# etzinis/sudo_rm_rf

Hardware: AMD Instinct MI355X
Metric: separated-seconds/sec (4s@8kHz mixtures), Improved-U16/512, 1->8 MI355X (higher is better)
Workload: dtype f32 (1x1 convs: fp32 operands split into bf16 hi+lo, 3 bf16 MFMAs per product, fp32 accumulate)

## Files before the change

### include/sudormrf_hip.h

```cpp
#ifndef SUDORMRF_HIP_H
#define SUDORMRF_HIP_H

#include <stddef.h>

#ifdef __cplusplus
extern "C" {
#endif

#define SRF_ABI_VERSION 19

#define SRF_STAT_BUCKETS 64

#define SRF_OK 0
#define SRF_EINVAL (-1)
#define SRF_EHIP (-2)
#define SRF_EWORKSPACE (-3)

#define SRF_VARIANT_IMPROVED 0
#define SRF_VARIANT_GROUPCOMM 1
#define SRF_VARIANT_CAUSAL 2

typedef struct srf_config {
  int variant;
  int in_audio_channels;
// ... 42 lines not shown
  SRF_DBG_GEMM_128_ONE_TILE_PER_BLOCK = 2048,
  SRF_DBG_WGRAD_NO_XCD_MAP = 4096,
  SRF_DBG_GEMM_256_SWAP_FORMS = 8192,
  SRF_DBG_TRAIN_BF16X3 = 16384,
  SRF_DBG_NO_FUSED_TAIL = 32768,
  SRF_DBG_BWD_NO_FUSED_HEAD = 1 << 16,
  SRF_DBG_PYR_PASS1_ROWS_PER_WAVE = 1 << 17,
  SRF_DBG_WGRAD_NO_WIDE_TILE = 1 << 18,
  SRF_DBG_WGRAD_128_MASKED = 1 << 19,
  SRF_DBG_WGRAD_SHORT_CHUNKS = 1 << 20,
  SRF_DBG_PAIR_PERSISTENT = 1 << 21,
  SRF_DBG_TAC_VALU = 1 << 22,
  SRF_DBG_PAIR_FULL_DRAIN = 1 << 23,
  SRF_DBG_TAC_GENERIC = 1 << 24,
  SRF_DBG_WGRAD_ONE_CHAIN_FOLD = 1 << 25,
  SRF_DBG_TAC_LANES_4TILES = 1 << 26,
  SRF_DBG_GEMM_128_POINTER_LOADS = 1 << 27,
  SRF_DBG_TRAIN_FWD_SPLIT_BF16 = 1 << 28,
  SRF_DBG_BWD_DW_CHUNKED = 1 << 29,
  SRF_DBG_BWD_GLN_SCALAR = 1 << 30,
  SRF_DBG_TRAIN_FWD_EXACT_MFMA = -2147483647 - 1
};
void srf_set_debug_flags(int flags);
#endif

int srf_plan_create(const srf_config* cfg, int batch, int T, srf_plan** out);
void srf_plan_destroy(srf_plan* plan);
size_t srf_plan_workspace_bytes(const srf_plan* plan);
int srf_plan_num_params(const srf_plan* plan);
int srf_plan_frames(const srf_plan* plan);
int srf_plan_padded_length(const srf_plan* plan);
int srf_plan_num_launches(const srf_plan* plan);

int srf_forward(const srf_plan* plan, const float* const* params, int num_params,
                const float* wav, float* out, void* workspace, size_t workspace_bytes, void* stream);

int srf_plan_ragged_supported(const srf_plan* plan);
size_t srf_plan_ragged_workspace_bytes(const srf_plan* plan);
int srf_forward_ragged(const srf_plan* plan, const float* const* params, int num_params, const float* wav,
                       const int* lengths , float* out, void* workspace, size_t workspace_bytes,
                       void* stream);

int srf_separate(const srf_plan* plan, const float* const* params, int num_params, const float* wav, float* out,
                 float* stats, int mixture_consistency, void* workspace, size_t workspace_bytes, void* stream);

int srf_separate_ragged(const srf_plan* plan, const float* const* params, int num_params, const float* wav,
// ... 316 lines not shown
```

### sudo_rm_rf_amd/_lib.py

```python
import ctypes as C
import os
import threading

import torch

_PKG = os.path.dirname(os.path.abspath(__file__))
LIB_PATH = os.environ.get("SRF_LIB") or os.path.join(_PKG, "libsudormrf_hip.so")
ABI_VERSION = 19
RAGGED_MAX_BATCH = 128
STAT_BUCKETS = 64

SRF_OK = 0
VARIANT_IMPROVED, VARIANT_GROUPCOMM, VARIANT_CAUSAL, VARIANT_ATTENTIVE, VARIANT_ATTENTIVE_V3, VARIANT_ORIGINAL = 0, 1, 2, 3, 4, 5
ATT_MAX_LEN = 5000
SOFTMAX_MASK_MAX_SOURCES = 16


class SrfError(RuntimeError):
    pass


class srf_config(C.Structure):
    _fields_ = [(n, C.c_int) for n in (
        "variant", "in_audio_channels", "out_channels", "in_channels", "num_blocks",
        "upsampling_depth", "enc_kernel_size", "enc_num_basis", "num_sources", "group_size")]


class srf_norm(C.Structure):
    _fields_ = [("sums", C.c_void_p), ("gamma", C.c_void_p), ("beta", C.c_void_p), ("prelu", C.c_void_p)]


class srf_stream_row(C.Structure):
    _fields_ = [("slot", C.c_int), ("n", C.c_int)]


_vp, _i, _sz, _l = C.c_void_p, C.c_int, C.c_size_t, C.c_long
_PROTOS = {
    "srf_abi_version": (_i, []),
    "srf_last_error": (C.c_char_p, []),
    "srf_set_kernel_mode": (None, [_i]),
    "srf_get_kernel_mode": (_i, []),
    "srf_profile_begin": (_i, [_vp]),
    "srf_profile_end": (_i, [_vp, C.POINTER(_i)]),
    "srf_profile_get": (_i, [_i, C.POINTER(C.c_char_p), C.POINTER(C.c_float)]),
    "srf_profile_timeline": (_i, [_i, C.POINTER(C.c_char_p), C.POINTER(C.c_float), C.POINTER(_i)]),
    "srf_plan_create": (_i, [C.POINTER(srf_config), _i, _i, C.POINTER(_vp)]),
    "srf_plan_destroy": (None, [_vp]),
    "srf_plan_workspace_bytes": (_sz, [_vp]),
    "srf_plan_num_params": (_i, [_vp]),
    "srf_plan_frames": (_i, [_vp]),
    "srf_plan_padded_length": (_i, [_vp]),
    "srf_plan_num_launches": (_i, [_vp]),
    "srf_forward": (_i, [_vp, C.POINTER(_vp), _i, _vp, _vp, _vp, _sz, _vp]),
    "srf_debug_fetch": (_i, [_vp, _vp, _i, _vp, _sz, _vp]),
    "srf_encoder": (_i, [_vp, _vp, _vp, _vp, _i, _i, _i, _i, _i, _i, _vp]),
    "srf_gln_stats": (_i, [_vp, _vp, _i, _l, _vp]),
    "srf_gln_apply": (_i, [_vp, _vp, C.POINTER(srf_norm), _i, _i, _i, _vp]),
    "srf_gln_apply_add": (_i, [_vp, _vp, _vp, C.POINTER(srf_norm), _i, _i, _i, _vp]),
    "srf_pw_conv": (_i, [_vp, _vp, _vp, _vp, _i, _i, _i, _i, C.POINTER(srf_norm), _vp, _vp, _i, _vp, _i, _vp]),
    "srf_set_debug_flags": (None, [_i]),
    "srf_packed_pw_weight_bytes": (_sz, [_i, _i]),
    "srf_pack_pw_weights": (_i, [C.POINTER(_vp), C.POINTER(_vp), C.POINTER(_i), C.POINTER(_i), _i, _vp]),
    "srf_pw_conv_packed": (_i, [_vp, _vp, _vp, _vp, _vp, _i, _i, _i, _i, C.POINTER(srf_norm), _vp, _vp, _i, _vp, _i, _vp]),
    "srf_pw_conv_pair_supported": (_i, [_i, _i, _i, _i, _i]),
    "srf_pw_conv_pair": (_i, [_vp, _vp, _vp, _vp, C.POINTER(srf_norm), _vp, _vp, _vp, _vp, _vp, _i, _i, _i, _i, _i, _vp]),
    "srf_pw_conv_pair_packed3_supported": (_i, [_i, _i, _i, _i, _i]),
    "srf_pw_conv_pair_packed3": (_i, [_vp, _vp, _vp, _vp, C.POINTER(srf_norm), _vp, _vp, _vp, _vp, _vp, _i, _i, _i, _i, _i, _vp]),
    "srf_packed3_pw_weight_bytes": (_sz, [_i, _i]),
    "srf_pack3_pw_weights": (_i, [C.POINTER(_vp), C.POINTER(_vp), C.POINTER(_i), C.POINTER(_i), _i, _vp]),
    "srf_pack3_forget": (None, [_vp]),
    "srf_pw_conv_packed3": (_i, [_vp, _vp, _vp, _vp, _vp, _i, _i, _i, _i, C.POINTER(srf_norm), _vp, _vp, _vp]),
    "srf_pit_sisdr_work_bytes": (_sz, [_i, _i]),
    "srf_perm_inv_sisdr_work_bytes": (_sz, [_i, _i]),
    "srf_perm_inv_sisdr": (_i, [_vp, _vp, _vp, _i, _i, _i, _i, C.c_double, _vp, _vp, _vp, _vp, _vp]),
    "srf_pit_sisdr_forward": (_i, [_vp, _vp, _i, _i, _i, C.c_float, _vp, _vp, _vp, _vp]),
    "srf_pit_sdr_forward": (_i, [_vp, _vp, _i, _i, _i, C.c_float, _i, _i, _i, _vp, _vp, _vp, _vp]),
    "srf_pit_sisdr_match": (_i, [_vp, _i, _i, _vp, _vp]),
    "srf_pit_sisdr_backward": (_i, [_vp, _vp, _i, _i, _i, C.c_float, _vp, _vp, _vp, _vp, _vp]),
    "srf_zeroref_snr_work_bytes": (_sz, [_i, _i, _i]),
    "srf_zeroref_snr_forward": (_i, [_vp, _vp, _i, _i, _i, _i, C.c_float, C.c_float, C.c_float, _vp, _vp, _vp, _vp, _vp]),
    "srf_zeroref_snr_backward": (_i, [_vp, _vp, _i, _i, _i, _vp, _vp, _i, _vp, _vp]),
    "srf_stab_sisdr_work_bytes": (_sz, [_i, _i]),
    "srf_stab_sisdr": (_i, [_vp, _vp, _i, _i, _i, _i, _i, _i, _i, C.c_double, _vp, _vp, _vp, _vp]),
# ... 197 lines not shown
```

### sudo_rm_rf_amd/csrc/srf_api.hip

```cpp
#include <string.h>

#include <atomic>
#include <mutex>
#include <new>
#include <vector>

#include "srf_plan.h"

static thread_local char g_err[512] = "";
static std::atomic<int> g_kernel_mode{0};

void srf_set_error(const char* fmt, ...) {
  va_list ap;
  va_start(ap, fmt);
  vsnprintf(g_err, sizeof(g_err), fmt, ap);
  va_end(ap);
}
static thread_local int g_kernel_mode_override = -1;
int srf_kernel_mode() { return g_kernel_mode_override >= 0 ? g_kernel_mode_override : g_kernel_mode.load(std::memory_order_relaxed); }
int srf_kernel_mode_override(int mode) {
  const int prev = g_kernel_mode_override;
  g_kernel_mode_override = mode;
  return prev;
}
static std::atomic<int> g_debug_flags{0};
int srf_debug_flags() { return g_debug_flags.load(std::memory_order_relaxed); }
extern "C" void srf_set_debug_flags(int f) { g_debug_flags.store(f, std::memory_order_relaxed); }

static std::mutex g_dev_mu;
static int g_dev_cus[SRF_MAX_DEVICES];
static long g_dev_occ[SRF_MAX_DEVICES][SRF_OCC_SLOTS];
static bool g_dev_occ_set[SRF_MAX_DEVICES][SRF_OCC_SLOTS];

int srf_current_device() {
  int dev = 0;
  return hipGetDevice(&dev) == hipSuccess ? dev : -1;
}
int srf_device_cus() {
  const int dev = srf_current_device();
  if (dev < 0 || dev >= SRF_MAX_DEVICES) return 256;
  std::lock_guard<std::mutex> lk(g_dev_mu);
  if (!g_dev_cus[dev]) {
    hipDeviceProp_t prop;
    g_dev_cus[dev] = hipGetDeviceProperties(&prop, dev) == hipSuccess ? prop.multiProcessorCount : 256;
  }
  return g_dev_cus[dev];
}
long srf_device_cached(int slot, long (*compute)(void*), void* arg) {
  const int dev = srf_current_device();
  if (dev < 0 || dev >= SRF_MAX_DEVICES || slot < 0 || slot >= SRF_OCC_SLOTS) return compute(arg);
// ... 398 lines not shown
}
static int step_pair(const Ragged* rg, const float* x, const void* w1_packed, const float* bias1, float* y, const srf_norm* in_norm,
                     const float* residual, const void* w2_packed, const float* bias2, float* y2, double* out_sums2, int Bt, int Cin1,
                     int Cmid, int Cout2, int L, void* stream) {
  return rg ? srf_pw_conv_pair_ragged(x, w1_packed, bias1, y, in_norm, residual, w2_packed, bias2, y2, out_sums2, Bt, Cin1, Cmid, Cout2,
                                      L, rg->frames, stream)
            : srf_pw_conv_pair(x, w1_packed, bias1, y, in_norm, residual, w2_packed, bias2, y2, out_sums2, Bt, Cin1, Cmid, Cout2, L,
                               stream);
}
static int step_tac(const Ragged* rg, const float* x, float* q, const float* const* params, int Bt, int G, int n, int H, int L,
                    double* out_sums, void* stream) {
  return rg ? srf_tac_ragged(x, q, params, Bt, G, n, H, L, out_sums, rg->frames, stream)
            : srf_tac(x, q, params, Bt, G, n, H, L, out_sums, stream);
}
static int step_preadd(const Ragged* rg, int G, const float* x, const float* q, const srf_norm* qnorm, float* u, const float* w,
                       const float* bias, float* y, int Bg, int Cin, int Cout, int L, double* out_sums, void* stream) {
  return rg ? srf_pw_conv_small_ragged(x, w, bias, y, Bg, Cin, Cout, L, nullptr, nullptr, out_sums, q, qnorm, u, rg->frames, G, stream)
            : srf_pw_conv_preadd(x, q, qnorm, u, w, bias, y, Bg, Cin, Cout, L, out_sums, (hipStream_t)stream);
}
static int step_pyramid(const Ragged* rg, int G, const float* y1, float* merged, const srf_norm* in_norm, const SrfBlock<const float>& b,
                        int Bg, int C, int L, int D, void* scratch, double* out_sums, void* stream) {
  return rg ? srf_pyramid_ragged_rows(y1, merged, in_norm, b.lv_w, b.lv_b, b.lv_g, b.lv_be, Bg, C, L, D, scratch, out_sums, rg->frames, G,
                                      stream)
            : srf_pyramid(y1, merged, in_norm, b.lv_w, b.lv_b, b.lv_g, b.lv_be, Bg, C, L, D, scratch, out_sums, stream);
}
static int step_overlap_add(const Ragged* rg, const float* z, float* out, int Bt, int Co, int K, int L, int T, int nparts,
                            const float* wav_stats, const float* wav, int mc, hipStream_t st) {
  return rg ? srf_overlap_add_launch(z, out, Bt, Co, K, L, T, nparts, wav_stats, wav, mc, st, &rg->lens_t, &rg->frames_t)
            : srf_overlap_add_launch(z, out, Bt, Co, K, L, T, nparts, wav_stats, wav, mc, st);
}

static int forward_walk(const srf_plan* p, const float* const* P, const float* wav, float* out, void* workspace,
                        const float* wav_stats, int mixture_consistency, const Ragged* rg, void* stream) {
  const srf_config& c = p->cfg;
  const bool gc = c.variant == SRF_VARIANT_GROUPCOMM;
  const int G = gc ? c.group_size : 1;
  const int D = c.upsampling_depth, U = c.num_blocks, N = c.enc_num_basis, K = c.enc_kernel_size;
  const int Bt = p->Bt, L = p->L, Bg = p->Bg, nB = p->nB, nC = p->nC;
  char* ws = (char*)workspace;
  hipStream_t st = (hipStream_t)stream;
  auto fptr = [&](size_t o) { return (float*)(ws + o); };
  double* stats = (double*)(ws + p->off_stats);
  int rc;

  rc = srf_zero_launch(stats, p->stats_bytes, st);
  if (rc) return rc;
  const bool use_pack = rg || plan_use_pack(p);
// ... 384 lines not shown
```

### sudo_rm_rf_amd/csrc/srf_common.h

```cpp
#pragma once
#include <hip/hip_runtime.h>
#include <stdarg.h>
#include <stdio.h>
#include <atomic>
#include <initializer_list>
#define SRF_DIAGNOSTICS 1
#include "../../include/sudormrf_hip.h"

#define SRF_WAVE 64
#define SRF_MAX_DEPTH 8

void srf_set_error(const char* fmt, ...);
int srf_kernel_mode();
int srf_kernel_mode_override(int mode);
int srf_debug_flags();
static inline bool srf_dbg(int mask) { return (srf_debug_flags() & mask) != 0; }
bool srf_profiling();
void srf_prof_hold(int delta);
void srf_prof_mark(const char* name, hipStream_t st);
#define SRF_MAX_DEVICES 64
int srf_current_device();
int srf_device_cus();
#define SRF_OCC_SLOTS 16
enum SrfOccSlot { SRF_OCC_PYR_PASS1_CH16 = 0, SRF_OCC_PYR_PASS1_CH32 = 1 };
long srf_device_cached(int slot, long (*compute)(void*), void* arg);

template <auto Kernel, typename... Args>
static inline bool srf_launch_lds(int max_lds, dim3 grid, dim3 block, size_t lds, hipStream_t st, const Args&... args) {
  static std::atomic<bool> raised[SRF_MAX_DEVICES];
  const int dev = srf_current_device();
  const bool known = dev >= 0 && dev < SRF_MAX_DEVICES;
  if (!known || !raised[dev].load(std::memory_order_acquire)) {
    if (hipFuncSetAttribute((const void*)Kernel, hipFuncAttributeMaxDynamicSharedMemorySize, max_lds) != hipSuccess) return false;
    if (known) raised[dev].store(true, std::memory_order_release);
  }
  hipLaunchKernelGGL(Kernel, grid, block, lds, st, args...);
  return true;
}

// ... 205 lines not shown
```

### sudo_rm_rf_amd/csrc/srf_internal.h

```cpp
#pragma once
#include "srf_common.h"

#define SRF_CAUSAL_TAPS 11
#define SRF_CAUSAL_KW 21

struct SrfFrames {
  int n[SRF_RAGGED_MAX_BATCH];
};
__device__ __forceinline__ int srf_frames_of(int) { return 0; }
__device__ __forceinline__ int srf_frames2_of(int) { return 0; }
template <typename... R>
__device__ __forceinline__ int srf_frames_of(int g, const SrfFrames& f, const R&...) { return f.n[g]; }
__device__ __forceinline__ int srf_frames2_of(int g, const SrfFrames&, const SrfFrames& f2) { return f2.n[g]; }
__device__ __forceinline__ int srf_frames_of(int row, const SrfFrames& f, int rows_per_example) { return f.n[row / rows_per_example]; }
int srf_frames_table(const char* what, const int* frames, int groups, int L, SrfFrames* out);

int srf_transpose_launch(const float* w, float* wt, int Ci, int M, hipStream_t st);
int srf_overlap_add_launch(const float* z, float* out, int Bt, int Co, int K, int L, int T, int nparts, const float* stats,
                           const float* wav, int mc, hipStream_t st, const SrfFrames* lens = nullptr,
                           const SrfFrames* frames = nullptr);
int srf_wav_stats_ragged_launch(const float* wav, const SrfFrames& lens, float* stats, int rows, int T, hipStream_t st);

int srf_zero_launch(void* p, size_t bytes, hipStream_t st);
int srf_decoder_impl(const float* v, const float* w, float* out, int Bt, int Ci, int Co, int K, int L, int T, float* scratch,
// ... 19 lines not shown

int srf_causal_scale_many(const float* const* src, float* const* dst, const long* n, const float* const* dscale,
                          const float* hscale, int count, hipStream_t st);

int srf_causal_merge_act(const float* const* d, const float* const* prelu, int D, float* y, int Bt, int C, int L, hipStream_t st);
int srf_causal_gain_fold(float* const* dw, float* const* db, const float* const* w, const float* const* b,
                         const float* const* gain, float* const* dgain, const float* alpha, int nw, int nb, int count,
                         hipStream_t st);
int srf_causal_enc_scatter(const float* src, float* dst, int N, int A, int K, hipStream_t st);
size_t srf_causal_prelu_bwd_scratch_floats();
int srf_causal_prelu_bwd(const float* gout, const float* x, const float* slope, float* gx, float* dslope, long n, float* scratch,
                         hipStream_t st);

template <typename T>
struct SrfBlock;
struct SrfSlots;
int srf_pyramid_per_level(const float* y1, float* const* lv, float* merged, const SrfBlock<const float>& b, const SrfSlots& s,
                          int Bg, int nC, int L, int D, void* stream);

bool srf_pyramid_reg_supported(int L, int D);
int srf_pyramid_impl(const float* y1, float* merged, const srf_norm* in_norm, const float* const* w,
                     const float* const* bias, const float* const* gamma, const float* const* beta, int groups, int C,
                     int L, int D, void* scratch, double* out_sums, float* const* lv_out, double* const* lv_sums,
                     void* stream);

void srf_pw_prefer_paired(bool on);
bool srf_pw_conv_preadd_supported(int Cin, int Cout, int L, const void* const* ptrs, int nptrs);
int srf_pw_conv_preadd(const float* x, const float* q, const srf_norm* qnorm, float* u, const float* w, const float* bias,
                       float* y, int Bt, int Cin, int Cout, int L, double* out_sums, hipStream_t st);
bool srf_mask_decode_supported(int Bt, int Cin, int Cout, int L, int M);
size_t srf_mask_decode_pack_bytes(int Cout);
int srf_mask_decode_pack(const float* wd, void* dst, int Ci, int M, hipStream_t st);
int srf_mask_decode(const float* x, const float* w, const void* w_packed, const float* bias, const float* prelu,
                    const float* mul, int mul_channels, const void* wd_packed, float* zpart, int Bt, int Cin, int Cout, int L,
                    int M, hipStream_t st);
int srf_pack_pw_weights_transposed(const float* const* w, void* const* packed, const int* Cout, const int* Cin, int n,
                                   hipStream_t st);
bool srf_pw_packed_only(const void* w_packed, const float* x, int Bt, int Cin, int Cout, int L);
bool srf_train_three_parts_override(bool on);
int srf_pw_data_grad(const float* g, const float* w, const void* wT_packed, float* wt, const float* zero_bias, float* gx, int Bt,
                     int Cin, int Cout, int L, const float* skip, hipStream_t st);

bool srf_x3w_supported(int Bt, int pro);
bool srf_x3w_shape_supported(int Cin, int Cout, int L);
size_t srf_x3w_packed_bytes(int Cout, int Cin);
int srf_x3w_pack_launch(const float* const* w, char* const* dst, const int* Cout, const int* Cin, int n, hipStream_t st);
int srf_x3w_pack2_launch(const float* const* w, char* const* dst, char* const* dst16, const int* Cout, const int* Cin, int n,
// ... 44 lines not shown
```

### sudo_rm_rf_amd/csrc/srf_pyr.h

```cpp
#pragma once
#include "srf_internal.h"

struct PyrRegArgs {
  const float* y1;
  float* d0;
  float* merged;
  SrfNormDev in_norm;
  const float* in_mr;
  double in_inv_count;
  const float* w[SRF_MAX_DEPTH];
  const float* bias[SRF_MAX_DEPTH];
  const float* gamma[SRF_MAX_DEPTH];
  const float* beta[SRF_MAX_DEPTH];
  const float* lvl;
  double* mom;
  double* out_sums;
  int rows;
  int rpw;
  int C, L, D, tiles, own;
  float* lv_out[SRF_MAX_DEPTH];
  int save = 0;
};

int srf_pyramid_reg_launch(PyrRegArgs a, bool moments, long rows, hipStream_t st, const SrfFrames* frames = nullptr,
                           int rows_per_example = 1);
```

### sudo_rm_rf_amd/csrc/srf_pyramid.hip

```cpp
#include "srf_pyr.h"

struct PyrArgs {
  const float* y1;
  float* merged;
  SrfNormDev in_norm;
  double in_inv_count;
  const float* w[SRF_MAX_DEPTH];
  const float* bias[SRF_MAX_DEPTH];
  const float* gamma[SRF_MAX_DEPTH];
  const float* beta[SRF_MAX_DEPTH];
  const float* lvl;
  const float* in_mr;
  float* d0;
  double* mom;
  double* out_sums;
  long rows;
  int C, L, D;
};

__device__ __forceinline__ float srf_dot5(const float* w, float x0, float x1, float x2, float x3, float x4,
                                          float init) {
  return fmaf(w[4], x4, fmaf(w[3], x3, fmaf(w[2], x2, fmaf(w[1], x1, fmaf(w[0], x0, init)))));
}

// ... 693 lines not shown
  t->TS = best;
  t->tiles = L / best;
  int h = 0;
  for (int k = SRF_MAX_DEPTH - 1; k >= 0; --k) {
    if (k >= D) {
      t->h[k] = 0;
      continue;
    }
    t->h[k] = (k == D - 1) ? 0 : 2 * h + 4;
    h = t->h[k];
  }
  const int len0 = best + 2 * t->h[0] + 8;
  int lv = 0;
  for (int k = 1; k < D; ++k) lv += (best >> k) + 2 * t->h[k] + 8;
  const int lenA = lv > len0 ? lv : len0;
  t->wave_floats = len0 + ((lenA + 3) & ~3) + 8 * SRF_MAX_DEPTH;
  return (size_t)t->wave_floats * 4 * sizeof(float) <= 64 * 1024;
}


int srf_pyramid_impl(const float* y1, float* merged, const srf_norm* in_norm, const float* const* w,
                     const float* const* bias, const float* const* gamma, const float* const* beta, int groups, int C,
                     int L, int D, void* scratch, double* out_sums, float* const* lv_out, double* const* lv_sums,
                     void* stream);

extern "C" int srf_pyramid(const float* y1, float* merged, const srf_norm* in_norm,
                           const float* const* w, const float* const* bias, const float* const* gamma,
                           const float* const* beta, int groups, int C, int L, int D, void* scratch,
                           double* out_sums, void* stream) {
  return srf_pyramid_impl(y1, merged, in_norm, w, bias, gamma, beta, groups, C, L, D, scratch, out_sums, nullptr, nullptr,
                          stream);
}

static int pyramid_run(const float* y1, float* merged, const srf_norm* in_norm, const float* const* w,
                       const float* const* bias, const float* const* gamma, const float* const* beta, int groups, int C,
                       int L, int D, void* scratch, double* out_sums, float* const* lv_out, double* const* lv_sums,
                       void* stream, const SrfFrames* frames, int rpe);
int srf_pyramid_impl(const float* y1, float* merged, const srf_norm* in_norm, const float* const* w,
                     const float* const* bias, const float* const* gamma, const float* const* beta, int groups, int C,
                     int L, int D, void* scratch, double* out_sums, float* const* lv_out, double* const* lv_sums,
                     void* stream) {
  return pyramid_run(y1, merged, in_norm, w, bias, gamma, beta, groups, C, L, D, scratch, out_sums, lv_out, lv_sums, stream,
                     nullptr, 1);
}

extern "C" int srf_pyramid_ragged_frames_ok(int frames, int L, int D) {
  if (D < 1 || D > SRF_MAX_DEPTH || frames < 1 || frames > L) return 0;
  if ((frames >> (D - 1)) < 8 || (frames % (1 << (D - 1))) != 0) return 0;
  return srf_pyramid_reg_supported(frames, D) ? 1 : 0;
}

extern "C" int srf_pyramid_ragged(const float* y1, float* merged, const srf_norm* in_norm, const float* const* w,
                                  const float* const* bias, const float* const* gamma, const float* const* beta, int groups,
                                  int C, int L, int D, void* scratch, double* out_sums, const int* frames, void* stream) {
  return srf_pyramid_ragged_rows(y1, merged, in_norm, w, bias, gamma, beta, groups, C, L, D, scratch, out_sums, frames, 1, stream);
}

extern "C" int srf_pyramid_ragged_rows(const float* y1, float* merged, const srf_norm* in_norm, const float* const* w,
                                       const float* const* bias, const float* const* gamma, const float* const* beta, int groups,
                                       int C, int L, int D, void* scratch, double* out_sums, const int* frames,
                                       int groups_per_example, void* stream) {
  SRF_CHECK_ARG(groups_per_example >= 1 && groups % groups_per_example == 0,
                "srf_pyramid_ragged: %d groups are not a whole number of examples of %d groups each", groups, groups_per_example);
  const int examples = groups / groups_per_example;
  SrfFrames fr;
  int rc = srf_frames_table("srf_pyramid_ragged", frames, examples, L, &fr);
// ... 145 lines not shown
```

### sudo_rm_rf_amd/csrc/srf_pyramid_reg.hip

```cpp
#include "srf_pyr.h"


template <int N>
__device__ __forceinline__ void srf_zero(float (&v)[N]) {
#pragma unroll
  for (int i = 0; i < N; ++i) v[i] = 0.f;
}

template <int N>
__device__ __forceinline__ void srf_conv_s1(const float (&x)[N], float (&out)[N], const float* w, float b) {
  const float l2 = srf_lane_up(x[N - 2]), l1 = srf_lane_up(x[N - 1]);
  const float r0 = srf_lane_down(x[0]), r1 = srf_lane_down(x[1]);
  float e[N + 4];
  e[0] = l2;
  e[1] = l1;
#pragma unroll
  for (int i = 0; i < N; ++i) e[i + 2] = x[i];
  e[N + 2] = r0;
  e[N + 3] = r1;
#pragma unroll
  for (int i = 0; i < N; ++i)
    out[i] = fmaf(w[4], e[i + 4], fmaf(w[3], e[i + 3], fmaf(w[2], e[i + 2], fmaf(w[1], e[i + 1], fmaf(w[0], e[i], b)))));
}

// ... 24 lines not shown
__device__ __forceinline__ void srf_acc_moments(const float (&v)[N], float& s, float& q) {
#pragma unroll
  for (int i = 0; i < N; ++i) {
    s += v[i];
    q = fmaf(v[i], v[i], q);
  }
}

struct LvCoef {
  float w[5], b, a, c;
};

template <int N>
__device__ __forceinline__ void srf_pyr_edges(double* m5, const float (&v)[N], int ci, int nchunks) {
  if (ci == 0) {
    m5[2] = (double)v[0];
    if (N >= 2) m5[3] = (double)v[N >= 2 ? 1 : 0];
  }
  if (N == 1 && ci == 1) m5[3] = (double)v[0];
  if (ci == nchunks - 1) m5[4] = (double)v[N - 1];
}

template <int CH>
__device__ __forceinline__ void srf_pyr_store_chunks(float4* strip, const float (&v)[CH], bool own, float* row_base,
                                                     int first_chunk, int cnt, int lane) {
  constexpr int NF = CH / 4, PF = NF + 1;
  const int j = lane - 2;
  if (own) {
#pragma unroll
    for (int i = 0; i < NF; ++i) strip[j * PF + i] = make_float4(v[4 * i], v[4 * i + 1], v[4 * i + 2], v[4 * i + 3]);
  }
  __builtin_amdgcn_fence(__ATOMIC_RELEASE, "wavefront");
  __builtin_amdgcn_wave_barrier();
  __builtin_amdgcn_fence(__ATOMIC_ACQUIRE, "wavefront");
  float4* dst = reinterpret_cast<float4*>(row_base + (size_t)first_chunk * CH);
#pragma unroll
  for (int it = 0; it < (60 * NF + 63) / 64; ++it) {
    const int f = it * 64 + lane;
    if (f < cnt * NF) dst[f] = strip[(f / NF) * PF + (f % NF)];
  }
  __builtin_amdgcn_fence(__ATOMIC_RELEASE, "wavefront");
  __builtin_amdgcn_wave_barrier();
  __builtin_amdgcn_fence(__ATOMIC_ACQUIRE, "wavefront");
}

template <int N>
__device__ __forceinline__ void srf_pyr_store_level(float* dst, const float (&v)[N]) {
  if constexpr (N >= 4) {
#pragma unroll
    for (int i = 0; i < N / 4; ++i)
      reinterpret_cast<float4*>(dst)[i] = make_float4(v[4 * i], v[4 * i + 1], v[4 * i + 2], v[4 * i + 3]);
  } else if constexpr (N == 2) {
    *reinterpret_cast<float2*>(dst) = make_float2(v[0], v[1]);
  } else {
    dst[0] = v[0];
  }
}

template <bool MOMENTS, int CH, bool PERSIST = MOMENTS, bool SAVE = false, typename... FR>
__global__ __launch_bounds__(256) void srf_pyramid_reg_kernel(PyrRegArgs a, FR... fr) {
  constexpr bool RAGGED = sizeof...(FR) != 0;
  __shared__ float4 pyr_strip[MOMENTS ? 1 : 4 * 60 * (CH / 4 + 1)];
  const int lane = threadIdx.x & 63;
  const int L = a.L, D = a.D, C = a.C;
  const int nchunks = L / CH;
  const int wave = __builtin_amdgcn_readfirstlane(threadIdx.x >> 6);
  int row, row_end, tile, g, c;
  if (PERSIST) {
    row = (blockIdx.x * 4 + wave) * a.rpw;
    if (row >= a.rows) return;
    row_end = min(row + a.rpw, a.rows);
    g = row / C;
    c = row - g * C;
    tile = 0;
  } else {
    c = blockIdx.x;
    g = blockIdx.z;
    row = g * C + c;
    row_end = row + 1;
    tile = blockIdx.y * 4 + wave;
    if (tile >= a.tiles) return;
  }
  const float* in_base = a.y1;
  int nch = nchunks, ntl = a.tiles;
  if constexpr (RAGGED) {
    nch = srf_frames_of(g, fr...) / CH;
    ntl = (nch + a.own - 1) / a.own;
    if (!MOMENTS && tile >= ntl) {
      float zv[CH];
      srf_zero(zv);
      const int ci0 = tile * a.own - 2 + lane;
      srf_pyr_store_chunks<CH>(pyr_strip + wave * (60 * (CH / 4 + 1)), zv, ci0 < nchunks && lane >= 2 && lane < 2 + a.own,
                               a.merged + (size_t)row * L, tile * a.own, min(a.own, nchunks - tile * a.own), lane);
      return;
    }
  }
  auto chunk_src = [&](int row_, int tile_, int nch_) {
    const int ci_ = min(max(tile_ * a.own - 2 + lane, 0), nch_ - 1);
    return reinterpret_cast<const float4*>(in_base + (size_t)row_ * L + ci_ * CH);
  };
  float s1[6], s2[6];
  int cur_g = -1;
  float in_mean = 0.f, in_rstd = 1.f;
  float4 pre[CH / 4];
  {
    const float4* src = chunk_src(row, tile, nch);
#pragma unroll
    for (int i = 0; i < CH / 4; ++i) pre[i] = src[i];
  }
  for (;;) {
  int nrow = row, ntile = tile + 1;
  int nnch = nch;
  if (ntile == ntl) {
    ntile = 0;
    nrow = row + 1;
    if constexpr (RAGGED) {
      if (c + 1 == C && nrow < row_end) nnch = srf_frames_of(g + 1, fr...) / CH;
    }
  }
  const bool last_task = !PERSIST || nrow >= row_end;
  const int ci = tile * a.own - 2 + lane;
  const bool valid = ci >= 0 && ci < nch;
  const bool own = valid && lane >= 2 && lane < 2 + a.own;

  LvCoef lc[SRF_MAX_DEPTH];
#pragma unroll
  for (int k = 0; k < SRF_MAX_DEPTH; ++k) {
    if (k < D && (CH >> k) >= 1) {
// ... 10 lines not shown
      }
    }
  }

  float x0[CH];
  {
    float sc = 1.f, sh = 0.f;
    if (a.in_norm.sums) {
      if (PERSIST) {
        if (g != cur_g) {
          const double inv_count = RAGGED ? 1.0 / ((double)C * (double)(nch * CH)) : a.in_inv_count;
          srf_finalize_stats(a.in_norm.sums, g, inv_count, in_mean, in_rstd);
          cur_g = g;
        }
      } else {
        in_mean = a.in_mr[2 * g];
        in_rstd = a.in_mr[2 * g + 1];
      }
      sc = a.in_norm.gamma[c] * in_rstd;
      sh = a.in_norm.beta[c] - in_mean * sc;
    }
    const bool act = a.in_norm.prelu != nullptr;
    const float slope = act ? a.in_norm.prelu[0] : 1.f;
    float o[CH];
#pragma unroll
    for (int i = 0; i < CH / 4; ++i) {
      const float4 v = pre[i];
      o[4 * i + 0] = v.x;
      o[4 * i + 1] = v.y;
      o[4 * i + 2] = v.z;
      o[4 * i + 3] = v.w;
    }
    const float scm = valid ? sc : 0.f, shm = valid ? sh : 0.f;
#pragma unroll
    for (int i = 0; i < CH; ++i) {
      float v = fmaf(o[i], scm, shm);
      if (act) v = srf_prelu(v, slope);
      o[i] = v;
    }
    srf_conv_s1<CH>(o, x0, lc[0].w, lc[0].b);
    if (SAVE && a.lv_out[0])
      srf_pyr_store_chunks<CH>(pyr_strip + (threadIdx.x >> 6) * (60 * (CH / 4 + 1)), x0, own, a.lv_out[0] + (size_t)row * L,
                               tile * a.own, min(a.own, nchunks - tile * a.own), lane);
    const float vmask = valid ? 1.f : 0.f;
    if (MOMENTS) {
#pragma unroll
      for (int i = 0; i < CH; ++i) x0[i] *= vmask;
    } else {
      srf_affine_mask<CH>(x0, lc[0].a, lc[0].c, valid);
    }
  }

  if (PERSIST) {
    const float4* src = chunk_src(last_task ? row : nrow, last_task ? tile : ntile, last_task ? nch : nnch);
#pragma unroll
    for (int i = 0; i < CH / 4; ++i) pre[i] = src[i];
  }

  float x1[CH / 2], x2[CH / 4], x3[CH / 8], x4[CH / 16], x5[CH / 32 > 0 ? CH / 32 : 1];
  srf_zero(x1);
  srf_zero(x2);
  srf_zero(x3);
  srf_zero(x4);
  srf_zero(x5);
  if (!PERSIST || tile == 0) {
// ... 92 lines not shown
        t = have ? v + t : v;
        have = true;
      }
      if (D > 2) {
        const float v = x2[i >> 2];
        t = have ? v + t : v;
        have = true;
      }
      if (D > 1) {
        const float v = x1[i >> 1];
        t = have ? v + t : v;
        have = true;
      }
      const float v = have ? x0[i] + t : x0[i];
      outv[i] = v;
      ms += v;
      mq = fmaf(v, v, mq);
    }
    if (!own) {
      ms = 0.f;
      mq = 0.f;
    }
    const bool own_st = RAGGED ? ci >= 0 && ci < nchunks && lane >= 2 && lane < 2 + a.own : own;
    srf_pyr_store_chunks<CH>(pyr_strip + wave * (60 * (CH / 4 + 1)), outv, own_st, a.merged + (size_t)row * L, tile * a.own,
                             min(a.own, nchunks - tile * a.own), lane);
    if (a.out_sums) {
      const double ds = srf_dpp_wave_sum((double)ms), dq = srf_dpp_wave_sum((double)mq);
      if (lane == 63) {
        double* dst = srf_stat_slot(a.out_sums, g, c * a.tiles + tile);
        atomicAdd(dst, ds);
        atomicAdd(dst + 1, dq);
      }
    }
  }
  if (last_task) break;
  if (ntile == 0 && ++c == C) {
    c = 0;
    ++g;
    if constexpr (RAGGED) {
      nch = nnch;
      ntl = (nch + a.own - 1) / a.own;
    }
  }
  row = nrow;
  tile = ntile;
  }
}
// ... 14 lines not shown
  const bool persist = moments && (frames || !srf_dbg(SRF_DBG_PYR_PASS1_NONPERSISTENT));
  long cw = 0;
  if (persist) {
    struct Q { int ch; } q{CH};
    cw = srf_device_cached(CH == 16 ? SRF_OCC_PYR_PASS1_CH16 : SRF_OCC_PYR_PASS1_CH32, [](void* p) -> long {
      const int ch = static_cast<Q*>(p)->ch;
      int per_cu = 0;
      const void* fn = ch == 16 ? (const void*)&srf_pyramid_reg_kernel<true, 16, true>
                                : (const void*)&srf_pyramid_reg_kernel<true, 32, true>;
      if (hipOccupancyMaxActiveBlocksPerMultiprocessor(&per_cu, fn, 256, 0) != hipSuccess || per_cu < 1) per_cu = 2;
      return (long)srf_device_cus() * per_cu * 4;
    }, &q);
  }
  dim3 grid;
  if (persist) {
    long nwaves = cw < rows ? cw : rows;
    a.rpw = srf_dbg(SRF_DBG_PYR_PASS1_ROWS_PER_WAVE) ? (int)((rows + nwaves - 1) / nwaves) : 1;
    nwaves = (rows + a.rpw - 1) / a.rpw;
    grid = dim3((unsigned)((nwaves + 3) / 4));
  } else {
    a.rpw = 1;
    grid = dim3((unsigned)a.C, (unsigned)((a.tiles + 3) / 4), (unsigned)(rows / a.C));
  }
  const bool save = !moments && a.save != 0;
  if (save)
    for (int k = 0; k < a.D; ++k)
      SRF_CHECK_ARG((a.lv_out[k] || (k == 0 && a.D > 1)) && srf_aligned16(a.lv_out[k]), "srf_pyramid: level output %d missing / unaligned", k);
  if (frames) {
    SRF_CHECK_ARG(!save, "srf_pyramid: the ragged form keeps no level outputs");
    const SrfFrames& fr = *frames;
    SRF_CHECK_ARG(rpe >= 1, "srf_pyramid: internal: rows per example");
    if (CH == 16 && moments) hipLaunchKernelGGL((srf_pyramid_reg_kernel<true, 16, true, false, SrfFrames, int>), grid, dim3(256), 0, st, a, fr, rpe);
    else if (CH == 16) hipLaunchKernelGGL((srf_pyramid_reg_kernel<false, 16, false, false, SrfFrames, int>), grid, dim3(256), 0, st, a, fr, rpe);
    else if (moments) hipLaunchKernelGGL((srf_pyramid_reg_kernel<true, 32, true, false, SrfFrames, int>), grid, dim3(256), 0, st, a, fr, rpe);
    else hipLaunchKernelGGL((srf_pyramid_reg_kernel<false, 32, false, false, SrfFrames, int>), grid, dim3(256), 0, st, a, fr, rpe);
    SRF_CHECK_LAUNCH(moments ? "pyramid_moments_ragged" : "pyramid_merge_ragged", st);
    return SRF_OK;
  }
  if (CH == 16) {
    if (moments && persist)
      hipLaunchKernelGGL((srf_pyramid_reg_kernel<true, 16, true>), grid, dim3(256), 0, st, a);
    else if (moments)
      hipLaunchKernelGGL((srf_pyramid_reg_kernel<true, 16, false>), grid, dim3(256), 0, st, a);
    else if (save)
      hipLaunchKernelGGL((srf_pyramid_reg_kernel<false, 16, false, true>), grid, dim3(256), 0, st, a);
    else
// ... 15 lines not shown
```

### sudo_rm_rf_amd/ops.py

```python
import contextlib
import ctypes as C
import enum
import weakref

import torch

from . import _lib


def _chk(*ts):
    dev = None
    for t in ts:
        if t is None:
            continue
        if t.device.type != "cuda":
            raise _lib.SrfError("sudo_rm_rf_amd ops need CUDA (ROCm) tensors; got %s" % t.device)
        if not t.is_contiguous():
            raise _lib.SrfError("tensor must be contiguous")
        dev = t.device
    return dev


def new_sums(groups, device):
    return torch.zeros((groups, _lib.STAT_BUCKETS, 2), dtype=torch.float64, device=device)
# ... 489 lines not shown
    GEMM_128_ONE_TILE_PER_BLOCK = 2048
    WGRAD_NO_XCD_MAP = 4096
    GEMM_256_SWAP_FORMS = 8192
    TRAIN_BF16X3 = 16384
    NO_FUSED_TAIL = 32768
    BWD_NO_FUSED_HEAD = 1 << 16
    PYR_PASS1_ROWS_PER_WAVE = 1 << 17
    WGRAD_NO_WIDE_TILE = 1 << 18
    WGRAD_128_MASKED = 1 << 19
    WGRAD_SHORT_CHUNKS = 1 << 20
    PAIR_PERSISTENT = 1 << 21
    TAC_VALU = 1 << 22
    PAIR_FULL_DRAIN = 1 << 23
    TAC_GENERIC = 1 << 24
    WGRAD_ONE_CHAIN_FOLD = 1 << 25
    TAC_LANES_4TILES = 1 << 26
    GEMM_128_POINTER_LOADS = 1 << 27
    TRAIN_FWD_SPLIT_BF16 = 1 << 28
    BWD_DW_CHUNKED = 1 << 29
    BWD_GLN_SCALAR = 1 << 30
    TRAIN_FWD_EXACT_MFMA = 1 << 31


_debug_flags = 0


def set_debug_flags(flags):
    global _debug_flags
    bits = int(flags) & 0xFFFFFFFF
    _lib.load().srf_set_debug_flags(bits - (1 << 32) if bits >> 31 else bits)
    _debug_flags = bits


@contextlib.contextmanager
def debug_flags(flags):
    prev = _debug_flags
    set_debug_flags(flags)
    try:
        yield
    finally:
        set_debug_flags(prev)


def set_kernel_mode(mode):
    _lib.load().srf_set_kernel_mode(int(mode))


def get_kernel_mode():
    return int(_lib.load().srf_get_kernel_mode())


class kernel_trace:

    def __init__(self, device):
# ... 20 lines not shown
```

Before: 22980.

## Load pyramid pass-2 input spans coalesced and transpose through LDS strips

For the 16-channel-chunk non-moments pyramid kernel, each wave now fetches its whole span of input chunks with coalesced float4 loads (non-temporal by default) and transposes them through a per-wave LDS strip, instead of each lane reading its own chunk. The strip per wave grows to 64 chunks. The non-ragged path now passes a rows-per-example value through, and a second debug-flag word with Python plumbing can restore per-lane or plain reads. The aim is less uncoalesced global traffic, in exchange for extra LDS round trips and wave barriers.

```diff
diff --git a/include/sudormrf_hip.h b/include/sudormrf_hip.h
--- a/include/sudormrf_hip.h
+++ b/include/sudormrf_hip.h
@@ -88,6 +88,15 @@
   SRF_DBG_TRAIN_FWD_EXACT_MFMA = -2147483647 - 1
 };
 void srf_set_debug_flags(int flags);
+enum srf_debug_flag2 {
+  SRF_DBG2_PYR_PASS2_LANE_LOADS = 1,
+  SRF_DBG2_PYR_PASS2_PLAIN_READS = 2
+};
+void srf_set_debug_flags2(int flags);
+int srf_pyramid_levels(const float* y1, float* merged, const srf_norm* in_norm, const float* const* w,
+                       const float* const* bias, const float* const* gamma, const float* const* beta, int groups,
+                       int C, int L, int D, void* scratch, double* out_sums, float* const* lv_out,
+                       double* const* lv_sums, void* stream);
 #endif
 
 int srf_plan_create(const srf_config* cfg, int batch, int T, srf_plan** out);
diff --git a/sudo_rm_rf_amd/_lib.py b/sudo_rm_rf_amd/_lib.py
--- a/sudo_rm_rf_amd/_lib.py
+++ b/sudo_rm_rf_amd/_lib.py
@@ -1,4 +1,5 @@
 import ctypes as C
+import enum
 import os
 import threading
 
@@ -18,6 +19,11 @@
 
 class SrfError(RuntimeError):
     pass
+
+
+class DebugFlag2(enum.IntFlag):
+    PYR_PASS2_LANE_LOADS = 1 << 32
+    PYR_PASS2_PLAIN_READS = 2 << 32
 
 
 class srf_config(C.Structure):
@@ -59,6 +65,9 @@
     "srf_gln_apply_add": (_i, [_vp, _vp, _vp, C.POINTER(srf_norm), _i, _i, _i, _vp]),
     "srf_pw_conv": (_i, [_vp, _vp, _vp, _vp, _i, _i, _i, _i, C.POINTER(srf_norm), _vp, _vp, _i, _vp, _i, _vp]),
     "srf_set_debug_flags": (None, [_i]),
+    "srf_set_debug_flags2": (None, [_i]),
+    "srf_pyramid_levels": (_i, [_vp, _vp, C.POINTER(srf_norm), C.POINTER(_vp), C.POINTER(_vp), C.POINTER(_vp),
+                               C.POINTER(_vp), _i, _i, _i, _i, _vp, _vp, C.POINTER(_vp), C.POINTER(_vp), _vp]),
     "srf_packed_pw_weight_bytes": (_sz, [_i, _i]),
     "srf_pack_pw_weights": (_i, [C.POINTER(_vp), C.POINTER(_vp), C.POINTER(_i), C.POINTER(_i), _i, _vp]),
     "srf_pw_conv_packed": (_i, [_vp, _vp, _vp, _vp, _vp, _i, _i, _i, _i, C.POINTER(srf_norm), _vp, _vp, _i, _vp, _i, _vp]),
diff --git a/sudo_rm_rf_amd/csrc/srf_api.hip b/sudo_rm_rf_amd/csrc/srf_api.hip
--- a/sudo_rm_rf_amd/csrc/srf_api.hip
+++ b/sudo_rm_rf_amd/csrc/srf_api.hip
@@ -26,6 +26,9 @@
 static std::atomic<int> g_debug_flags{0};
 int srf_debug_flags() { return g_debug_flags.load(std::memory_order_relaxed); }
 extern "C" void srf_set_debug_flags(int f) { g_debug_flags.store(f, std::memory_order_relaxed); }
+static std::atomic<int> g_debug_flags2{0};
+int srf_debug_flags2() { return g_debug_flags2.load(std::memory_order_relaxed); }
+extern "C" void srf_set_debug_flags2(int f) { g_debug_flags2.store(f, std::memory_order_relaxed); }
 
 static std::mutex g_dev_mu;
 static int g_dev_cus[SRF_MAX_DEVICES];
@@ -470,7 +473,7 @@
                         int Bg, int C, int L, int D, void* scratch, double* out_sums, void* stream) {
   return rg ? srf_pyramid_ragged_rows(y1, merged, in_norm, b.lv_w, b.lv_b, b.lv_g, b.lv_be, Bg, C, L, D, scratch, out_sums, rg->frames, G,
                                       stream)
-            : srf_pyramid(y1, merged, in_norm, b.lv_w, b.lv_b, b.lv_g, b.lv_be, Bg, C, L, D, scratch, out_sums, stream);
+            : srf_pyramid_impl(y1, merged, in_norm, b.lv_w, b.lv_b, b.lv_g, b.lv_be, Bg, C, L, D, scratch, out_sums, nullptr, nullptr, stream, G);
 }
 static int step_overlap_add(const Ragged* rg, const float* z, float* out, int Bt, int Co, int K, int L, int T, int nparts,
                             const float* wav_stats, const float* wav, int mc, hipStream_t st) {
diff --git a/sudo_rm_rf_amd/csrc/srf_common.h b/sudo_rm_rf_amd/csrc/srf_common.h
--- a/sudo_rm_rf_amd/csrc/srf_common.h
+++ b/sudo_rm_rf_amd/csrc/srf_common.h
@@ -15,6 +15,8 @@
 int srf_kernel_mode_override(int mode);
 int srf_debug_flags();
 static inline bool srf_dbg(int mask) { return (srf_debug_flags() & mask) != 0; }
+int srf_debug_flags2();
+static inline bool srf_dbg2(int mask) { return (srf_debug_flags2() & mask) != 0; }
 bool srf_profiling();
 void srf_prof_hold(int delta);
 void srf_prof_mark(const char* name, hipStream_t st);
diff --git a/sudo_rm_rf_amd/csrc/srf_internal.h b/sudo_rm_rf_amd/csrc/srf_internal.h
--- a/sudo_rm_rf_amd/csrc/srf_internal.h
+++ b/sudo_rm_rf_amd/csrc/srf_internal.h
@@ -65,7 +65,7 @@
 int srf_pyramid_impl(const float* y1, float* merged, const srf_norm* in_norm, const float* const* w,
                      const float* const* bias, const float* const* gamma, const float* const* beta, int groups, int C,
                      int L, int D, void* scratch, double* out_sums, float* const* lv_out, double* const* lv_sums,
-                     void* stream);
+                     void* stream, int rows_per_example = 1);
 
 void srf_pw_prefer_paired(bool on);
 bool srf_pw_conv_preadd_supported(int Cin, int Cout, int L, const void* const* ptrs, int nptrs);
diff --git a/sudo_rm_rf_amd/csrc/srf_pyr.h b/sudo_rm_rf_amd/csrc/srf_pyr.h
--- a/sudo_rm_rf_amd/csrc/srf_pyr.h
+++ b/sudo_rm_rf_amd/csrc/srf_pyr.h
@@ -20,6 +20,8 @@
   int C, L, D, tiles, own;
   float* lv_out[SRF_MAX_DEPTH];
   int save = 0;
+  int lane_loads = 0;
+  int plain_reads = 0;
 };
 
 int srf_pyramid_reg_launch(PyrRegArgs a, bool moments, long rows, hipStream_t st, const SrfFrames* frames = nullptr,
diff --git a/sudo_rm_rf_amd/csrc/srf_pyramid.hip b/sudo_rm_rf_amd/csrc/srf_pyramid.hip
--- a/sudo_rm_rf_amd/csrc/srf_pyramid.hip
+++ b/sudo_rm_rf_amd/csrc/srf_pyramid.hip
@@ -739,7 +739,7 @@
 int srf_pyramid_impl(const float* y1, float* merged, const srf_norm* in_norm, const float* const* w,
                      const float* const* bias, const float* const* gamma, const float* const* beta, int groups, int C,
                      int L, int D, void* scratch, double* out_sums, float* const* lv_out, double* const* lv_sums,
-                     void* stream);
+                     void* stream, int rows_per_example);
 
 extern "C" int srf_pyramid(const float* y1, float* merged, const srf_norm* in_norm,
                            const float* const* w, const float* const* bias, const float* const* gamma,
@@ -747,6 +747,14 @@
                            double* out_sums, void* stream) {
   return srf_pyramid_impl(y1, merged, in_norm, w, bias, gamma, beta, groups, C, L, D, scratch, out_sums, nullptr, nullptr,
                           stream);
+}
+
+extern "C" int srf_pyramid_levels(const float* y1, float* merged, const srf_norm* in_norm, const float* const* w,
+                                  const float* const* bias, const float* const* gamma, const float* const* beta, int groups,
+                                  int C, int L, int D, void* scratch, double* out_sums, float* const* lv_out,
+                                  double* const* lv_sums, void* stream) {
+  SRF_CHECK_ARG(lv_out && lv_sums, "srf_pyramid_levels: null pointer");
+  return srf_pyramid_impl(y1, merged, in_norm, w, bias, gamma, beta, groups, C, L, D, scratch, out_sums, lv_out, lv_sums, stream);
 }
 
 static int pyramid_run(const float* y1, float* merged, const srf_norm* in_norm, const float* const* w,
@@ -756,9 +764,9 @@
 int srf_pyramid_impl(const float* y1, float* merged, const srf_norm* in_norm, const float* const* w,
                      const float* const* bias, const float* const* gamma, const float* const* beta, int groups, int C,
                      int L, int D, void* scratch, double* out_sums, float* const* lv_out, double* const* lv_sums,
-                     void* stream) {
+                     void* stream, int rows_per_example) {
   return pyramid_run(y1, merged, in_norm, w, bias, gamma, beta, groups, C, L, D, scratch, out_sums, lv_out, lv_sums, stream,
-                     nullptr, 1);
+                     nullptr, rows_per_example);
 }
 
 extern "C" int srf_pyramid_ragged_frames_ok(int frames, int L, int D) {
diff --git a/sudo_rm_rf_amd/csrc/srf_pyramid_reg.hip b/sudo_rm_rf_amd/csrc/srf_pyramid_reg.hip
--- a/sudo_rm_rf_amd/csrc/srf_pyramid_reg.hip
+++ b/sudo_rm_rf_amd/csrc/srf_pyramid_reg.hip
@@ -70,6 +70,45 @@
 }
 
 template <int CH>
+constexpr bool srf_pyr_span_loads = CH == 16;
+template <int CH>
+constexpr int srf_pyr_strip_chunks = srf_pyr_span_loads<CH> ? 64 : 60;
+template <int CH>
+__device__ __forceinline__ float4* srf_pyr_strip_of(float4* strips, int wave) {
+  return strips + wave * (srf_pyr_strip_chunks<CH> * (CH / 4 + 1));
+}
+
+__device__ __forceinline__ void srf_pyr_strip_sync() {
+  __builtin_amdgcn_fence(__ATOMIC_RELEASE, "wavefront");
+  __builtin_amdgcn_wave_barrier();
+  __builtin_amdgcn_fence(__ATOMIC_ACQUIRE, "wavefront");
+}
+
+template <int CH, bool NT>
+__device__ __forceinline__ void srf_pyr_fetch_span(float4 (&pre)[CH / 4], const float* row_base, int first_chunk, int nch, int lane) {
+  constexpr int NF = CH / 4;
+#pragma unroll
+  for (int it = 0; it < NF; ++it) {
+    const int f = it * 64 + lane;
+    const int ci = min(max(first_chunk + f / NF, 0), nch - 1);
+    pre[it] = srf_ld4<NT>(row_base + (size_t)ci * CH + (f % NF) * 4);
+  }
+}
+template <int CH>
+__device__ __forceinline__ void srf_pyr_transpose_span(float4* strip, float4 (&pre)[CH / 4], int lane) {
+  constexpr int NF = CH / 4, PF = NF + 1;
+#pragma unroll
+  for (int it = 0; it < NF; ++it) {
+    const int f = it * 64 + lane;
+    strip[(f / NF) * PF + (f % NF)] = pre[it];
+  }
+  srf_pyr_strip_sync();
+#pragma unroll
+  for (int i = 0; i < NF; ++i) pre[i] = strip[lane * PF + i];
+  srf_pyr_strip_sync();
+}
+
+template <int CH>
 __device__ __forceinline__ void srf_pyr_store_chunks(float4* strip, const float (&v)[CH], bool own, float* row_base,
                                                      int first_chunk, int cnt, int lane) {
   constexpr int NF = CH / 4, PF = NF + 1;
@@ -78,18 +117,14 @@
 #pragma unroll
     for (int i = 0; i < NF; ++i) strip[j * PF + i] = make_float4(v[4 * i], v[4 * i + 1], v[4 * i + 2], v[4 * i + 3]);
   }
-  __builtin_amdgcn_fence(__ATOMIC_RELEASE, "wavefront");
-  __builtin_amdgcn_wave_barrier();
-  __builtin_amdgcn_fence(__ATOMIC_ACQUIRE, "wavefront");
+  srf_pyr_strip_sync();
   float4* dst = reinterpret_cast<float4*>(row_base + (size_t)first_chunk * CH);
 #pragma unroll
   for (int it = 0; it < (60 * NF + 63) / 64; ++it) {
     const int f = it * 64 + lane;
     if (f < cnt * NF) dst[f] = strip[(f / NF) * PF + (f % NF)];
   }
-  __builtin_amdgcn_fence(__ATOMIC_RELEASE, "wavefront");
-  __builtin_amdgcn_wave_barrier();
-  __builtin_amdgcn_fence(__ATOMIC_ACQUIRE, "wavefront");
+  srf_pyr_strip_sync();
 }
 
 template <int N>
@@ -108,11 +143,12 @@
 template <bool MOMENTS, int CH, bool PERSIST = MOMENTS, bool SAVE = false, typename... FR>
 __global__ __launch_bounds__(256) void srf_pyramid_reg_kernel(PyrRegArgs a, FR... fr) {
   constexpr bool RAGGED = sizeof...(FR) != 0;
-  __shared__ float4 pyr_strip[MOMENTS ? 1 : 4 * 60 * (CH / 4 + 1)];
+  __shared__ float4 pyr_strips[MOMENTS ? 1 : 4 * srf_pyr_strip_chunks<CH> * (CH / 4 + 1)];
   const int lane = threadIdx.x & 63;
   const int L = a.L, D = a.D, C = a.C;
   const int nchunks = L / CH;
   const int wave = __builtin_amdgcn_readfirstlane(threadIdx.x >> 6);
+  float4* const pyr_strip = MOMENTS ? pyr_strips : srf_pyr_strip_of<CH>(pyr_strips, wave);
   int row, row_end, tile, g, c;
   if (PERSIST) {
     row = (blockIdx.x * 4 + wave) * a.rpw;
@@ -138,7 +174,7 @@
       float zv[CH];
       srf_zero(zv);
       const int ci0 = tile * a.own - 2 + lane;
-      srf_pyr_store_chunks<CH>(pyr_strip + wave * (60 * (CH / 4 + 1)), zv, ci0 < nchunks && lane >= 2 && lane < 2 + a.own,
+      srf_pyr_store_chunks<CH>(pyr_strip, zv, ci0 < nchunks && lane >= 2 && lane < 2 + a.own,
                                a.merged + (size_t)row * L, tile * a.own, min(a.own, nchunks - tile * a.own), lane);
       return;
     }
@@ -151,7 +187,22 @@
   int cur_g = -1;
   float in_mean = 0.f, in_rstd = 1.f;
   float4 pre[CH / 4];
-  {
+  constexpr bool SPAN = !MOMENTS && srf_pyr_span_loads<CH>;
+  [[maybe_unused]] bool span_loads = false;
+  if constexpr (SPAN) {
+    span_loads = !a.lane_loads;
+    const float* rb = span_loads ? in_base + (size_t)row * L : reinterpret_cast<const float*>(chunk_src(row, tile, nch));
+    if (span_loads) {
+      if (a.plain_reads) srf_pyr_fetch_span<CH, false>(pre, rb, tile * a.own - 2, nch, lane);
+      else srf_pyr_fetch_span<CH, true>(pre, rb, tile * a.own - 2, nch, lane);
+    } else if (a.plain_reads) {
+#pragma unroll
+      for (int i = 0; i < CH / 4; ++i) pre[i] = srf_ld4<false>(rb + 4 * i);
+    } else {
+#pragma unroll
+      for (int i = 0; i < CH / 4; ++i) pre[i] = srf_ld4<true>(rb + 4 * i);
+    }
+  } else {
     const float4* src = chunk_src(row, tile, nch);
 #pragma unroll
     for (int i = 0; i < CH / 4; ++i) pre[i] = src[i];
@@ -208,6 +259,9 @@
     }
     const bool act = a.in_norm.prelu != nullptr;
     const float slope = act ? a.in_norm.prelu[0] : 1.f;
+    if constexpr (SPAN) {
+      if (span_loads) srf_pyr_transpose_span<CH>(pyr_strip, pre, lane);
+    }
     float o[CH];
 #pragma unroll
     for (int i = 0; i < CH / 4; ++i) {
@@ -226,7 +280,7 @@
     }
     srf_conv_s1<CH>(o, x0, lc[0].w, lc[0].b);
     if (SAVE && a.lv_out[0])
-      srf_pyr_store_chunks<CH>(pyr_strip + (threadIdx.x >> 6) * (60 * (CH / 4 + 1)), x0, own, a.lv_out[0] + (size_t)row * L,
+      srf_pyr_store_chunks<CH>(pyr_strip, x0, own, a.lv_out[0] + (size_t)row * L,
                                tile * a.own, min(a.own, nchunks - tile * a.own), lane);
     const float vmask = valid ? 1.f : 0.f;
     if (MOMENTS) {
@@ -365,7 +419,7 @@
       mq = 0.f;
     }
     const bool own_st = RAGGED ? ci >= 0 && ci < nchunks && lane >= 2 && lane < 2 + a.own : own;
-    srf_pyr_store_chunks<CH>(pyr_strip + wave * (60 * (CH / 4 + 1)), outv, own_st, a.merged + (size_t)row * L, tile * a.own,
+    srf_pyr_store_chunks<CH>(pyr_strip, outv, own_st, a.merged + (size_t)row * L, tile * a.own,
                              min(a.own, nchunks - tile * a.own), lane);
     if (a.out_sums) {
       const double ds = srf_dpp_wave_sum((double)ms), dq = srf_dpp_wave_sum((double)mq);
@@ -426,6 +480,8 @@
     a.rpw = 1;
     grid = dim3((unsigned)a.C, (unsigned)((a.tiles + 3) / 4), (unsigned)(rows / a.C));
   }
+  a.lane_loads = rpe > 1 || srf_dbg2(SRF_DBG2_PYR_PASS2_LANE_LOADS);
+  a.plain_reads = rpe > 1 || srf_dbg2(SRF_DBG2_PYR_PASS2_PLAIN_READS);
   const bool save = !moments && a.save != 0;
   if (save)
     for (int k = 0; k < a.D; ++k)
diff --git a/sudo_rm_rf_amd/ops.py b/sudo_rm_rf_amd/ops.py
--- a/sudo_rm_rf_amd/ops.py
+++ b/sudo_rm_rf_amd/ops.py
@@ -535,14 +535,20 @@
     TRAIN_FWD_EXACT_MFMA = 1 << 31
 
 
+DebugFlag2 = _lib.DebugFlag2
+
 _debug_flags = 0
 
 
 def set_debug_flags(flags):
     global _debug_flags
-    bits = int(flags) & 0xFFFFFFFF
+    flags = int(flags)
+    bits = flags & 0xFFFFFFFF
+    if flags < 0:
+        flags = bits
     _lib.load().srf_set_debug_flags(bits - (1 << 32) if bits >> 31 else bits)
-    _debug_flags = bits
+    _lib.load().srf_set_debug_flags2((flags >> 32) & 0x7FFFFFFF)
+    _debug_flags = flags & 0x7FFFFFFFFFFFFFFF
 
 
 @contextlib.contextmanager
```

New measurement: 23150 (median of 6 runs). Within noise of the previous version (+0.8%).
